# RWKV/rwkv.cpp

Measured on AMD Instinct MI355X. Metric: tokens/sec single-stream decode, higher is better.
Workload: dtype int8 x int4 dot, f32 accumulate (Q4_0 weights, Q8_0 activations); f16 head; 1 GPU; RWKV-6-World-7B Q4_0 single-stream greedy decode, state resident in HBM; layers=32, n_embed=4096, n_vocab=65536, parallelism=1 GPU, persist_kind=2

## Files before the change

### rwkv.cpp_amd/csrc/ring_geom.h

```cpp
#pragma once

#include <stdint.h>

#if defined(__HIPCC__)
#define RG_HD __host__ __device__ inline
#else
#define RG_HD inline
#endif

namespace rwkvmi {

constexpr int RG_NBLK = 256;
constexpr int RG_NC = 6;
constexpr int RG_CHUNK = 1024;

enum { RG_W1 = 0, RG_C = 1, RG_DW1 = 2, RG_E = 3, RG_FK = 4, RG_FR = 5, RG_G = 6, RG_NPHASE = 7 };

struct RingShape {
    int D, F, R5, DR;
    int qs, scb, qhb;
    int bal = 0;
};

constexpr int RG_BAL_C_N[3] = {5, 7, 4};
// ... 89 lines not shown
        if (j0 < c.n[p]) return c.off[p] + j0 * c.rec[p];
    }
    return RG_NONE;
}

constexpr int RG_HSTEPS = 8;
constexpr uint32_t RG_HREC = RG_HSTEPS * 1024;
struct RingHead { int hg, chunks, passes; uint32_t bytes; };
RG_HD RingHead rg_head(int n_vocab, int K) {
    RingHead h;
    h.hg = n_vocab / (RG_NBLK * 16);
    h.chunks = K / 32 / RG_HSTEPS;
    h.passes = (h.hg + RG_NC - 1) / RG_NC;
    h.bytes = (uint32_t) h.hg * (uint32_t) h.chunks * RG_HREC;
    return h;
}
RG_HD int rg_head_npc(const RingHead & h, int pass) { const int r = h.hg - RG_NC * pass; return r < RG_NC ? r : RG_NC; }
RG_HD uint32_t rg_head_off(const RingHead & h, int pass, int chunk, int cons) {
    return ((uint32_t) (RG_NC * pass * h.chunks) + (uint32_t) (chunk * rg_head_npc(h, pass) + cons)) * RG_HREC;
}

RG_HD int rg_x_rows(const RingShape & s, int cons) { const int n = rg_rows_e(s); return cons < n ? (n - cons + RG_NC - 1) / RG_NC : 0; }

}
```

### rwkv.cpp_amd/csrc/ring_v6.hip

```cpp
#include "persist.h"
#include "ring_geom.h"

namespace rwkvmi {

struct R6Cu { unsigned long long base; unsigned chunks, chunks_head; unsigned layer_bytes, pad; };

struct R6P {
    const M6Layer * layers; int n_layers;
    const unsigned char * arena;
    const float * w2b;
    float * x;
    float * x_out;
    const float * sin; float * sout; long long state_stride;
    void * xch; unsigned xch_bytes;
    int tl, act5, rkvg, dl, yq, xatt, kq, xffn;
    int act_stride;
    unsigned * ctl;
    const unsigned char * stream; const R6Cu * cus;
    int layer0, layers_total;
    int F, DR, R, H;
    int head_wg0;
    unsigned ring_bytes, mirror_bytes;
    int inflight, thin;
    int look;
    int look_g;
    int hthin;
    int nap;
    int burst;
    int dbg;
    float * logits; long long lnout_w, lnout_b; int n_vocab;
    const unsigned * tok; unsigned * next_tok; const void * emb; int emb_f16; long long ln0_w, ln0_b; int am;
    long long * trace; int trace_layer;
};

enum { FL_LANDED = 0, FL_SWB = 1, FL_SWE = 2 , FL_DONE = 4 , FL_GX = 12, FL_GACT = 13, FL_GYQ = 14, FL_GKQ = 15,
       FL_RED1 = 16, FL_RED2 = 17, FL_PRO = 18, FL_KEYS = 19,
       FL_HX = 20, FL_HACT = 21, FL_HYQ = 22, FL_HKQ = 23, FL_HTL = 24 ,
       FL_PROX = 25 ,
       FL_HWB = 26, FL_HWE = 27 ,
       FL_XRQ = 28 ,
       FL_AM = 29 , FL_WORDS = 32 };

struct R6Lds { size_t x, q1, q2, u, tl, bc, red, out, dl, misc, fl, ring, fixed; };
__host__ __device__ inline R6Lds r6_lds(int D, int F) {
    R6Lds o; size_t p = 0;
    auto take = [&](size_t n) { const size_t r = p; p += (n + 15) / 16 * 16; return r; };
    o.x = take((size_t) D * 4); o.q1 = take(qvec_bytes(D)); o.q2 = take(qvec_bytes(D));
    const size_t ua = 3 * ((qvec_bytes(D) + 15) / 16 * 16), ub = qvec_bytes(F);
    o.u = take(ua > ub ? ua : ub);
    o.tl = take(5 * 64 * 4); o.bc = take(64 * 16); o.red = take(2 * 256 * 8); o.out = take(64 * 4); o.dl = take(qvec_bytes(256)); o.misc = take(64);
    o.fl = take(FL_WORDS * 4);
    p = (p + 1023) / 1024 * 1024;
    o.ring = p; o.fixed = p;
    return o;
}

__device__ __forceinline__ unsigned fl_ld(unsigned * f) { return __builtin_amdgcn_readfirstlane(__hip_atomic_load(f, __ATOMIC_RELAXED, __HIP_MEMORY_SCOPE_WORKGROUP)); }
__device__ __forceinline__ void fl_st(unsigned * f, unsigned v) { asm volatile("" ::: "memory"); if ((threadIdx.x & 63) == 0) __hip_atomic_store(f, v, __ATOMIC_RELAXED, __HIP_MEMORY_SCOPE_WORKGROUP); }
__device__ __forceinline__ void fl_add(unsigned * f, unsigned v) { asm volatile("" ::: "memory"); if ((threadIdx.x & 63) == 0) (void) __hip_atomic_fetch_add(f, v, __ATOMIC_RELAXED, __HIP_MEMORY_SCOPE_WORKGROUP); }

__device__ __forceinline__ bool lds_backoff(Poll & pl, unsigned spin) {
    if ((spin & 1023u) == 1023u) {
        if (__hip_atomic_load(pl.ctl + 1, __ATOMIC_RELAXED, __HIP_MEMORY_SCOPE_AGENT) != 0u) pl.dead = true;
        else if (spin > 60000000u) { __hip_atomic_store(pl.ctl + 1, 2u, __ATOMIC_RELAXED, __HIP_MEMORY_SCOPE_AGENT); pl.dead = true; }
    }
    __builtin_amdgcn_s_sleep(1);
    return pl.dead;
}
__device__ __forceinline__ void fl_wait(Poll & pl, unsigned * f, unsigned want) {
    for (unsigned spin = 0;; spin++) {
        if (fl_ld(f) >= want || pl.dead) break;
        if (lds_backoff(pl, spin)) break;
    }
    asm volatile("" ::: "memory");
}

template <int FMT> struct RBlk { wv4i q[QF<FMT>::QS / 16]; unsigned qh, sc; };
template <int FMT, int R, int U> struct RawRec { RBlk<FMT> raw[U][R]; };
// ... 557 lines not shown
        for (int o = 32; o > 0; o >>= 1) { const float ov = __shfl_xor(best, o, WAVE); const int oi = __shfl_xor(bi, o, WAVE); am_merge(best, bi, ov, oi); }
    }

#ifndef R6_DMA_OFFSET_BOTH
#define R6_DMA_OFFSET_BOTH 1
#endif
    template <bool NT>
    static __device__ __forceinline__ void dma_quad(unsigned long long sbase, unsigned voff, unsigned m0dst) {
        unsigned keep;
#if R6_DMA_OFFSET_BOTH
#define R6_QUAD(POL) "s_mov_b32 %0, m0\n\ts_mov_b32 m0, %3\n\ts_nop 0\n\t" \
                     "global_load_lds_dwordx4 %1, %2" POL "\n\tglobal_load_lds_dwordx4 %1, %2 offset:1024" POL "\n\t" \
                     "global_load_lds_dwordx4 %1, %2 offset:2048" POL "\n\tglobal_load_lds_dwordx4 %1, %2 offset:3072" POL "\n\ts_mov_b32 m0, %0"
#else
#define R6_QUAD(POL) "s_mov_b32 %0, m0\n\ts_mov_b32 m0, %3\n\ts_nop 0\n\t" \
                     "global_load_lds_dwordx4 %1, %2" POL "\n\ts_add_u32 m0, m0, 0x400\n\ts_nop 0\n\tglobal_load_lds_dwordx4 %1, %2 offset:1024" POL "\n\t" \
                     "s_add_u32 m0, m0, 0x400\n\ts_nop 0\n\tglobal_load_lds_dwordx4 %1, %2 offset:2048" POL "\n\t" \
                     "s_add_u32 m0, m0, 0x400\n\ts_nop 0\n\tglobal_load_lds_dwordx4 %1, %2 offset:3072" POL "\n\ts_mov_b32 m0, %0"
#endif
        if constexpr (NT) asm volatile(R6_QUAD(" nt") : "=&s"(keep) : "v"(voff), "s"(sbase), "s"(m0dst) : "memory");
        else asm volatile(R6_QUAD("") : "=&s"(keep) : "v"(voff), "s"(sbase), "s"(m0dst) : "memory");
#undef R6_QUAD
    }
    static __device__ __forceinline__ void wait_vm(int w) {
        switch (w >> 2) {
            case 0:  asm volatile("s_waitcnt vmcnt(0)" ::: "memory"); break;
            case 1:  asm volatile("s_waitcnt vmcnt(4)" ::: "memory"); break;
            case 2:  asm volatile("s_waitcnt vmcnt(8)" ::: "memory"); break;
            case 3:  asm volatile("s_waitcnt vmcnt(12)" ::: "memory"); break;
            case 4:  asm volatile("s_waitcnt vmcnt(16)" ::: "memory"); break;
            case 5:  asm volatile("s_waitcnt vmcnt(20)" ::: "memory"); break;
            case 6:  asm volatile("s_waitcnt vmcnt(24)" ::: "memory"); break;
            case 7:  asm volatile("s_waitcnt vmcnt(28)" ::: "memory"); break;
            case 8:  asm volatile("s_waitcnt vmcnt(32)" ::: "memory"); break;
            case 9:  asm volatile("s_waitcnt vmcnt(36)" ::: "memory"); break;
            case 10: asm volatile("s_waitcnt vmcnt(40)" ::: "memory"); break;
            case 11: asm volatile("s_waitcnt vmcnt(44)" ::: "memory"); break;
            case 12: asm volatile("s_waitcnt vmcnt(48)" ::: "memory"); break;
            default: asm volatile("s_waitcnt vmcnt(52)" ::: "memory"); break;
        }
    }
    static __device__ __forceinline__ void loader_main(const R6P & p, const Lds & l, int lane) {
        const int wave = 0;
        const R6Cu cu = p.cus[blockIdx.x];
        unsigned total_ = p.logits ? cu.chunks_head : cu.chunks;
        if (p.n_layers != p.layers_total) {
            const unsigned long long bytes = (unsigned long long) p.n_layers * cu.layer_bytes + (p.logits ? (unsigned long long) rg_head(p.n_vocab, D).bytes : 0ull);
            total_ = (unsigned) ((bytes + 4 * RG_CHUNK - 1) / (4 * RG_CHUNK)) * 4u;
        }
        const unsigned total = __builtin_amdgcn_readfirstlane(total_);
        const unsigned long long src0 = (unsigned long long) p.stream + cu.base + (unsigned long long) p.layer0 * cu.layer_bytes;
        const unsigned RB = __builtin_amdgcn_readfirstlane(p.ring_bytes), MIR = __builtin_amdgcn_readfirstlane(p.mirror_bytes);
        const unsigned ring_m0 = __builtin_amdgcn_readfirstlane((unsigned) (size_t) (__attribute__((address_space(3))) unsigned char *) l.ring);
        const unsigned voff = (unsigned) lane * 16u;
        const int w_norm = __builtin_amdgcn_readfirstlane(p.inflight) & ~3, w_thin = __builtin_amdgcn_readfirstlane(p.thin) & ~3, w_hint = __builtin_amdgcn_readfirstlane(p.hthin) & ~3;
        Poll pl{p.ctl, false};
        unsigned issued = 0, roff = 0, landed = 0;
        unsigned min_done = 0, thin = 0;
        int level = 0;
        const unsigned burst = (unsigned) __builtin_amdgcn_readfirstlane(p.burst);
        const unsigned s_lo = __builtin_amdgcn_readfirstlane((unsigned) src0), s_hi = __builtin_amdgcn_readfirstlane((unsigned) (src0 >> 32));
        const int li = p.trace_layer;
        R6STAMP(0);
        unsigned stalls = 0, rounds = 0;
        unsigned long long sb = ((unsigned long long) s_hi << 32) | s_lo;
        unsigned * const fland = l.fl + FL_LANDED;
        long long * const lsamp = (p.trace && (blockIdx.x == 0 || blockIdx.x == 131)) ? p.trace + (size_t) gridDim.x * 8 * 32 + (blockIdx.x == 0 ? 0 : 2048) : nullptr;
        const unsigned samp_lo = (unsigned) p.trace_layer * cu.layer_bytes, samp_hi = samp_lo + cu.layer_bytes;
        unsigned nsamp = 0;
        for (unsigned spin = 0; issued < total;) {
            const unsigned lim0 = min_done >= total * 1024u ? total : ((min_done + RB) >> 12) << 2;
            const unsigned lim = lim0 < total ? lim0 : total;
            asm volatile("" ::: "memory");
            const v4u da = *reinterpret_cast<const v4u *>(l.fl + FL_DONE), db = *reinterpret_cast<const v4u *>(l.fl + FL_DONE + 4);
            const v4u dh = *reinterpret_cast<const v4u *>(l.fl);
            const uint2 dw = *reinterpret_cast<const uint2 *>(l.fl + FL_HWB);
            const int w = thin == 1u ? w_thin : (thin == 2u ? w_hint : w_norm);
            rounds++;
            if (lsamp && nsamp < 512u && issued * 1024u + 4096u > samp_lo && landed * 1024u < samp_hi) {
                if (lane == 0) {
                    long long * o = lsamp + (size_t) nsamp * 4;
                    o[0] = (long long) __builtin_amdgcn_s_memrealtime(); o[1] = (long long) issued * 1024 - samp_lo; o[2] = (long long) landed * 1024 - samp_lo;
                    o[3] = (long long) min_done - samp_lo;
                }
                nsamp++;
            }
            if (issued < lim) {
                spin = 0;
                unsigned n = (lim - issued) >> 2;
                n = n < burst ? n : burst;
                for (unsigned k = 0; k < n; k++) {
                    if (roff < MIR) { dma_quad<false>(sb, voff, ring_m0 + RB + roff); dma_quad<true>(sb, voff, ring_m0 + roff); level += 8; }
                    else { dma_quad<true>(sb, voff, ring_m0 + roff); level += 4; }
                    sb += 4096ull;
                    roff += 4096u; roff = roff >= RB ? 0u : roff;
                }
                issued += 4u * n;
                if (level > w) { wait_vm(w); level = w; }
            } else {
                stalls++;
                if (level > 0) { const int x = (level - 1) & ~3; wait_vm(x); level = x; }
                else if (lds_backoff(pl, spin++)) break;
            }
            {
                const unsigned ld = issued > (unsigned) level ? issued - (unsigned) level : 0u;
                if (ld > landed) { landed = ld; asm volatile("" ::: "memory"); __hip_atomic_store(fland, landed, __ATOMIC_RELAXED, __HIP_MEMORY_SCOPE_WORKGROUP); }
            }
            {
                unsigned m = da.x < da.y ? da.x : da.y; m = m < da.z ? m : da.z; m = m < da.w ? m : da.w;
                m = m < db.x ? m : db.x; m = m < db.y ? m : db.y; m = m < db.z ? m : db.z; m = m < db.w ? m : db.w;
                min_done = __builtin_amdgcn_readfirstlane(m);
                thin = __builtin_amdgcn_readfirstlane(dh.y != dh.z ? 1u : (dw.x != dw.y ? 2u : 0u));
            }
        }
        wait_vm(0);
        fl_st(l.fl + FL_LANDED, total);
        R6STAMP(1);
        if (p.trace && lane == 0) {
            p.trace[((long long) blockIdx.x * 8 + wave) * 32 + 2] = (long long) stalls;
            p.trace[((long long) blockIdx.x * 8 + wave) * 32 + 3] = (long long) rounds;
        }
    }

    struct Cons {
        RingCu cu;
        unsigned lbase;
        unsigned next_block;
        unsigned RB;
        unsigned ring_lds;
        unsigned landed;
        int c, lane;
        int dbg;
        unsigned look;
        long long waited;
    };
    template <int T, int TE> struct Unroll {
        template <typename F> static __device__ __forceinline__ void run(F && f) { f(std::integral_constant<int, T>{}); Unroll<T + 1, TE>::run(f); }
    };
    template <int TE> struct Unroll<TE, TE> { template <typename F> static __device__ __forceinline__ void run(F &&) {} };

    template <int PH, int R, int U, int NP> struct Pre {
        static constexpr int PH_ = PH, R_ = R, U_ = U, NP_ = NP;
        static constexpr unsigned RECB = (unsigned) (U * R * 64) * (QF<FMT>::QS + (QF<FMT>::HM ? 4 : 2) + (QF<FMT>::QH ? 4 : 0));
        RawRec<FMT, R, U> w[NP];
        unsigned have;
        unsigned cnt;
        unsigned pos, ro;
        unsigned after;
        unsigned base;
    };
    template <int PH, int T>
    static __device__ __forceinline__ unsigned ownj(const Cons & cs) {
// ... 18 lines not shown
        const unsigned nxt = rg_next_own_in_layer(cs.cu, cs.c, PH + 1);
        pre.after = __builtin_amdgcn_readfirstlane(nxt != RG_NONE ? cs.lbase + nxt : cs.next_block);
#pragma unroll
        for (int i = 0; i < NP; i++) rec_reserve<FMT, R, U>(pre.w[i]);
    }
    template <int T, int PH, int R, int U, int NP, bool WAIT = true>
    static __device__ __forceinline__ bool rec_take(Cons & cs, Poll & pl, const Lds & l, Pre<PH, R, U, NP> & pre, bool block) {
        constexpr unsigned RECB = recb<R, U>(), STRIDE = NC * RECB;
        const unsigned need = (pre.pos + RECB + 1023u) >> 10;
        if (cs.landed < need) {
            cs.landed = fl_ld(l.fl + FL_LANDED);
            if (cs.landed < need) {
                if (!block) return false;
                const long long t0 = (long long) __builtin_readcyclecounter();
                for (unsigned spin = 0;; spin++) {
                    cs.landed = fl_ld(l.fl + FL_LANDED);
                    if (cs.landed >= need || pl.dead) break;
                    if (lds_backoff(pl, spin)) break;
                }
                cs.waited += (long long) __builtin_readcyclecounter() - t0;
            }
        }
        asm volatile("" ::: "memory");
        rec_load<FMT, R, U>(pre.w[T % NP], cs.ring_lds, pre.ro, opq(cs.lane));
        asm volatile("" ::: "memory");
        const bool last = pre.have + 1u >= pre.cnt;
        unsigned nxt;
        if constexpr (balph<PH>()) nxt = pre.base + ownj<PH, T + 1>(cs) * RECB; else nxt = pre.pos + STRIDE;
        __hip_atomic_store(l.fl + FL_DONE + 2 + cs.c, last ? pre.after : nxt, __ATOMIC_RELAXED, __HIP_MEMORY_SCOPE_WORKGROUP);
        if constexpr (WAIT) rec_wait<FMT, R, U>(pre.w[T % NP]);
        pre.have += 1u;
        pre.ro += nxt - pre.pos; pre.pos = nxt;
        pre.ro = pre.ro >= cs.RB ? pre.ro - cs.RB : pre.ro;
        if constexpr (!balph<PH>() && STRIDE > 32768u) { pre.ro = pre.ro >= cs.RB ? pre.ro - cs.RB : pre.ro; pre.ro = pre.ro >= cs.RB ? pre.ro - cs.RB : pre.ro; }
        return true;
    }
#ifndef R6_PRE_MASK
#define R6_PRE_MASK 255
#endif
#ifndef R6_PRE_MASK_SMALL
#define R6_PRE_MASK_SMALL 255
#endif
    static constexpr int PRE_MASK = EPT > 4 ? R6_PRE_MASK : R6_PRE_MASK_SMALL;
    template <int PA_, int RA, int UA, int NA, int PB_, int RB_, int UB_, int NB_, int PC_, int RC, int UC, int NC_>
    static __device__ __forceinline__ void hint_take(Cons & cs, Poll & pl, const Lds & l, xrsrc xr, int unit, unsigned tag, unsigned * go, unsigned gen, int nap,
                                                     bool on_a, Pre<PA_, RA, UA, NA> & a, bool on_b, Pre<PB_, RB_, UB_, NB_> & b, bool on_c, Pre<PC_, RC, UC, NC_> & c3, bool no_handover = false) {
// ... 112 lines not shown
#ifndef R6_NPC
#define R6_NPC (Q8 ? 3 : (Q5 ? 5 : 6))
#endif
#ifndef R6_NPE
#define R6_NPE 3
#endif
#ifndef R6_NPK
#define R6_NPK ((PRE_MASK & 128) ? (Q8 ? 2 : (Q5 ? 4 : 5)) : (Q8 ? 3 : (Q5 ? 5 : 6)))
#endif
#ifndef R6_NPG
#define R6_NPG (Q8 ? 1 : 3)
#endif
    static constexpr int NPC = npcap((PRE_MASK & 1) ? R6_NPC : (Q8 ? 1 : 2), TFC);
    static constexpr int NPE = npcap((PRE_MASK & 2) ? R6_NPE : (Q8 ? 1 : 2), TFE);
    static constexpr int NPK = npcap((PRE_MASK & 4) ? R6_NPK : (Q8 ? 1 : 2), TFK);
    static constexpr int NPR = npcap((PRE_MASK & 128) ? 3 : (Q8 ? 1 : 2), TFE);
    static constexpr int NPG = npcap((PRE_MASK & 8) ? R6_NPG : 1, TFE);
#ifndef R6_G_PRE_OLD
#define R6_G_PRE_OLD 0
#endif
    static constexpr int rec_regs(int R, int U) { return U * R * (QF<FMT>::QS / 4 + 1 + (QF<FMT>::QH ? 1 : 0)); }
    static constexpr bool G_PRE = R6_G_PRE_OLD ? sizeof(RawRec<FMT, 1, UF>) <= 48 * 4 : rec_regs(1, UF) <= 48;

    static __device__ __forceinline__ void consumer_main(const R6P & p, const Lds & l, int lane, int wave, unsigned base) {
        const int blk = blockIdx.x;
        const int c = wave - 2;
        const bool pro = c < 4 || SHI > 0;
        const int F = p.F, nbF = F / 32;
        Poll pl{p.ctl, false, p.xch, R6_SWATCH == 1};
        const M6Arena ar{p.arena};
        const xrsrc xr = make_xrsrc(p.xch, p.xch_bytes);
        const RingShape sh = shape(p);
        Cons cs;
        cs.cu = rg_cu(sh, blk); cs.lbase = 0; cs.landed = 0; cs.RB = __builtin_amdgcn_readfirstlane(p.ring_bytes); cs.ring_lds = __builtin_amdgcn_readfirstlane((unsigned) (size_t) (__attribute__((address_space(3))) unsigned char *) l.ring); cs.c = c; cs.lane = lane; cs.dbg = __builtin_amdgcn_readfirstlane(p.dbg); cs.look = (unsigned) __builtin_amdgcn_readfirstlane(p.look); cs.waited = 0;
        const int mat = (blk * (4 * D / NBLK)) / D;
        const int cbase = (blk * (4 * D / NBLK)) % D;
        const bool has_dw1 = blk < p.DR;

        const unsigned first_own = rg_next_own_in_layer(cs.cu, c, 0);
        const RingHead hd = rg_head(p.n_vocab, D);
        const unsigned hbase = (unsigned) p.n_layers * cs.cu.layer_bytes;
        const unsigned head_first = (p.logits && c < hd.hg) ? hbase + rg_head_off(hd, 0, 0, c) : 0xFFFFFFFFu;
        float xown[XT], rrow[XT];
#pragma unroll
        for (int t = 0; t < XT; t++) { const int row = c + NC * t; xown[t] = row < RE ? p.x[blk * RE + row] : 0.0f; rrow[t] = 0.0f; }
        const bool emb_in = p.tok != nullptr;
        const unsigned eg = emb_in ? 1u : 0u;
        if (emb_in && c < 4) embed_ln0(p, pl, l, ar, c * 64 + opq(lane), opq(lane));
#ifndef R6_LATE_PARAMS
#define R6_LATE_PARAMS 2
#endif
        constexpr bool PA_EARLY = R6_LATE_PARAMS == 0 || (R6_LATE_PARAMS == 2 && (PRE_MASK & 16) == 0);
        constexpr bool PF_EARLY = R6_LATE_PARAMS == 0 || (R6_LATE_PARAMS == 2 && (PRE_MASK & 4) == 0);
        PA pa; PF pf;
        if (PA_EARLY) issue_pa(pa, ar, p.layers[0], p.sin, c, opq(lane));

        for (int li = 0; li < p.n_layers; li++) {
            const M6Layer & L = p.layers[li];
            const float * sin_l = p.sin + (long long) li * p.state_stride;
            float * sout_l = p.sout + (long long) li * p.state_stride;
            const unsigned tagL = base + (unsigned) li * 8u;
            const unsigned g1 = (unsigned) li + 1u;
            cs.lbase = (unsigned) li * cs.cu.layer_bytes;
            cs.next_block = li + 1 < p.n_layers ? cs.lbase + cs.cu.layer_bytes + first_own : head_first;
            R6STAMP(0);
            if (p.trace && li == p.trace_layer && lane == 0) p.trace[((long long) blockIdx.x * 8 + wave) * 32 + 23] = cs.waited;
            unsigned havepk = 0u;
            Pre<RG_W1, 1, UD, 1> pw;
            pre_begin<RG_W1>(cs, pw);
            Pre<RG_C, 2, UD, NPC> pc;
            pre_begin<RG_C>(cs, pc);
            {
                const bool first = li == 0;
                watch_begin(l);
                hint_take(cs, pl, l, xr, p.xffn + ((blk * 37 + c * 211) & 1023), tagL - 8u + SLOT_XFFN, l.fl + FL_HX, 2u * li + 1u, p.nap, (PRE_MASK & 16) != 0 && !first, pw,
                          (PRE_MASK & 16) != 0 && !first, pc, first);
                watch_end(l);
                if (R6_LATE_PARAMS == 2 && !PA_EARLY) { issue_pa(pa, ar, L, sin_l, c, opq(lane)); __builtin_amdgcn_sched_barrier(0); }
                sweep_begin(l);
                gather_x(pl, xr, p.xffn, tagL - 8u + SLOT_XFFN, c, opq(lane), l.x, first ? p.x : nullptr, first && emb_in);
            }
            gather_meet(pl, l.fl + FL_GX, 2u * li + 1u);
            sweep_end(l);
            R6STAMP(1);
            {
                const bool take = li == 0 && emb_in;
#pragma unroll
                for (int t = 0; t < XT; t++) { const int row = c + NC * t; const float v = l.x[blk * RE + (row < RE ? row : 0)]; xown[t] = take ? v : xown[t]; }
            }
            if (R6_LATE_PARAMS == 1) { issue_pa(pa, ar, L, sin_l, c, opq(lane)); __builtin_amdgcn_sched_barrier(0); }
            if (pro) prologue_A(pl, l, pa, sout_l, blk == 0, c, opq(lane), 2u * li + 1u, eg);
            prologue_wait(pl, l, 2u * li + 1u);
            R6STAMP(2);
            havepk |= pw.have;
            rows<RG_W1, 1, UD, 0, 1>(cs, pl, l, qvec_at(l.q1, D), nb, pw, [&](auto, int j, const float (&res)[1]) {
                if (lane == 0) tg_store(xr, p.tl + blk + NBLK * j, __float_as_uint(det_tanhf(res[0])), 0u, 0u, 0u, tagL + SLOT_TL);
            });
            R6STAMP(3);
            Pre<RG_E, 1, UD, NPE> pe;
            pre_begin<RG_E>(cs, pe);
            {
                const int img = (0x4213 >> (4 * mat)) & 0xF;
// ... 61 lines not shown
            sweep_end(l);
            R6STAMP(8);
            if (R6_LATE_PARAMS == 1) { issue_pf(pf, ar, L, sin_l, c, opq(lane)); __builtin_amdgcn_sched_barrier(0); }
            if (pro) prologue_F(pl, l, pf, sout_l, blk == 0, c, opq(lane), 2u * li + 2u, eg);
            prologue_wait(pl, l, 2u * li + 2u);
            R6STAMP(9); R6RSTAMP(28);
            if (p.trace && li == p.trace_layer && lane == 0) p.trace[((long long) blockIdx.x * 8 + wave) * 32 + 21] = (long long) fl_ld(l.fl + FL_LANDED) * 1024ll - (long long) (cs.lbase + cs.cu.off[RG_FK]);
            havepk |= (pk.have << 12) | (pr.have << 16);
            rows<RG_FK, 2, UD, TFK, NPK, TMK>(cs, pl, l, qvec_at(l.q1, D), nb, pk, [&](auto, int j, const float (&res)[2]) {
                const float v = lane == 1 ? res[1] : res[0];
                const float t = v > 0.0f ? v : 0.0f;
                if (lane < 2) l.out[2 * j + lane] = t * t;
            });
            fl_add(l.fl + FL_KEYS, 1u);
            if constexpr (DEFER_XR) {
                if (pro) quant_xr(l, c, opq(lane));
                fl_wait(pl, l.fl + FL_XRQ, (unsigned) (SHI > 0 ? NC : 4) * g1);
            }
            R6STAMP(10);
            rows<RG_FR, 1, UD, RE / NC, NPR>(cs, pl, l, qvec_at(l.q2, D), nb, pr, [&](auto tc, int, const float (&res)[1]) {
                constexpr int t = decltype(tc)::value;
                rrow[t] = res[0];
            });
            R6STAMP(11); R6RSTAMP(29);
            Pre<RG_G, 1, UF, NPG> pg;
            pre_begin<RG_G>(cs, pg);
            watch_begin(l);
            { const unsigned lk = cs.look; cs.look = (unsigned) __builtin_amdgcn_readfirstlane(p.look_g);
              hint_take(cs, pl, l, xr, p.kq + ((blk * 5 + c * 173) & 511), tagL + SLOT_KQ, l.fl + FL_HKQ, g1, p.nap, (PRE_MASK & 8) != 0 && G_PRE, pg);
              cs.look = lk; }
            watch_end(l);
            sweep_begin(l);
            gather_qvec<KSL>(pl, xr, p.kq, F, tagL + SLOT_KQ, c, opq(lane), l.kq);
            gather_meet(pl, l.fl + FL_GKQ, g1);
            sweep_end(l);
            R6STAMP(12); R6RSTAMP(30);
            if (p.trace && li == p.trace_layer && lane == 0) p.trace[((long long) blockIdx.x * 8 + wave) * 32 + 22] = (long long) fl_ld(l.fl + FL_LANDED) * 1024ll - (long long) (cs.lbase + cs.cu.off[RG_G]);
            havepk |= pg.have << 20;
            rows<RG_G, 1, UF, RE / NC, NPG>(cs, pl, l, qvec_at(l.kq, F), nbF, pg, [&](auto tc, int j, const float (&res)[1]) {
                constexpr int t = decltype(tc)::value;
                const float gte = sigmoid_f(rrow[t]) * res[0];
                xown[t] = xown[t] + gte;
                if (li == p.n_layers - 1 && lane == 0) p.x_out[blk * RE + j] = xown[t];
            });
            if (lane == 0) tg_store(xr, p.xffn + blk * NC + c, __float_as_uint(xown[0]), __float_as_uint(xown[XT > 1 ? 1 : 0]), __float_as_uint(xown[XT > 2 ? 2 : 0]), 0u, tagL + SLOT_XFFN);
            R6STAMP(13); R6RSTAMP(14);
            if (p.trace && li == p.trace_layer && lane == 0) { p.trace[((long long) blockIdx.x * 8 + wave) * 32 + 25] = cs.waited; p.trace[((long long) blockIdx.x * 8 + wave) * 32 + 15] = (long long) havepk; }
            __builtin_amdgcn_sched_barrier(0);
            if (PA_EARLY) {
                const int nl = li + 1 < p.n_layers ? li + 1 : li;
                issue_pa(pa, ar, p.layers[nl], p.sin + (long long) nl * p.state_stride, c, opq(lane));
            }
            __builtin_amdgcn_sched_barrier(0);
        }
        if (p.logits) head_phase(p, l, cs, pl, xr, ar, hd, hbase, lane, wave, base, eg);
    }

    static __device__ __forceinline__ void head_phase(const R6P & p, const Lds & l, Cons & cs, Poll & pl, xrsrc xr, const M6Arena & ar, const RingHead & hd,
                                                      unsigned hbase, int lane, int wave, unsigned base, unsigned eg) {
        const int blk = blockIdx.x, c = cs.c, li = p.n_layers;
        const unsigned tagL = base + (unsigned) li * 8u;
        const int pt = c * 64 + lane;
        R6STAMP(0); R6RSTAMP(16);
        watch_begin(l);
        gather_hint(pl, xr, p.xffn + ((blk * 37 + c * 211) & 1023), tagL - 8u + SLOT_XFFN, l.fl + FL_HX, 2u * li + 1u, p.nap);
        watch_end(l);
        sweep_begin(l);
        gather_x(pl, xr, p.xffn, tagL - 8u + SLOT_XFFN, c, opq(lane), l.x);
        gather_meet(pl, l.fl + FL_GX, 2u * li + 1u);
        sweep_end(l);
        R6STAMP(1);
        if (c < 4) {
            const float scale = ln_stats(pl, l, pt, lane, 2u * li + 1u + eg);
            const float * lw = ar.f(p.lnout_w), * lb = ar.f(p.lnout_b);
#pragma unroll
            for (int u = 0; u < (D + 1023) / 1024; u++) {
                const int i = pt * 4 + u * 1024;
                if (i >= D) break;
                const float4 xc = *reinterpret_cast<const float4 *>(l.x + i);
                const float4 w4 = *reinterpret_cast<const float4 *>(lw + i), b4 = *reinterpret_cast<const float4 *>(lb + i);
                const float xs[4] = {xc.x, xc.y, xc.z, xc.w}, ws[4] = {w4.x, w4.y, w4.z, w4.w}, bs[4] = {b4.x, b4.y, b4.z, b4.w};
                float y[4];
#pragma unroll
                for (int j = 0; j < 4; j++) { const float a = xs[j] * scale; const float aw = a * ws[j]; y[j] = round_f16(aw + bs[j]); }
                *reinterpret_cast<float4 *>(l.x + i) = make_float4(y[0], y[1], y[2], y[3]);
            }
            fl_add(l.fl + FL_PRO, 1u);
        }
        fl_wait(pl, l.fl + FL_PRO, 4u * (2u * li + 1u));
        R6STAMP(2);
// ... 67 lines not shown
        fl_add(l.fl + FL_AM, 1u);
        R6STAMP(7); R6RSTAMP(17);
        if (p.trace && li == p.trace_layer && lane == 0) p.trace[((long long) blockIdx.x * 8 + wave) * 32 + 21] = waited;
    }

    static __device__ __forceinline__ void comm_main(const R6P & p, const Lds & l, int lane, unsigned base) {
        const int wave = 1;
        const int blk = blockIdx.x;
        const int g = NC;
        const int F = p.F, DR = p.DR, R = p.R, H = p.H;
        const int nbF = F / 32;
        Poll pl{p.ctl, false, p.xch, R6_SWATCH != 0};
        const M6Arena ar{p.arena};
        const xrsrc xr = make_xrsrc(p.xch, p.xch_bytes);
        const int mat = (blk * (4 * D / NBLK)) / D;
        const bool has_dw1 = blk < DR;
        const int hw0 = __builtin_amdgcn_readfirstlane(p.head_wg0);
        const bool d_has = blk >= hw0 && blk < hw0 + H;
        const int d_head = blk - hw0;
        const int gpb = (nbF + NBLK - 1) / NBLK;
        constexpr int NCH = 5 * (D / 64);
        const int b_extra = NCH - NBLK;
        const int b_chunk2 = (b_extra > 0 && blk >= NBLK / 4 && blk < NBLK / 4 + b_extra) ? NBLK + (blk - NBLK / 4) : -1;

        for (int li = 0; li < p.n_layers; li++) {
            const M6Layer & L = p.layers[li];
            const float * sin_l = p.sin + (long long) li * p.state_stride;
            float * sout_l = p.sout + (long long) li * p.state_stride;
            const unsigned tagL = base + (unsigned) li * 8u;
            const unsigned g1 = (unsigned) li + 1u;
            R6STAMP(0);
            {
                const bool first = li == 0;
                watch_begin(l);
                if (!first) gather_hint(pl, xr, p.xffn + ((blk * 37 + g * 211) & 1023), tagL - 8u + SLOT_XFFN, l.fl + FL_HX, 2u * li + 1u, p.nap);
                watch_end(l);
                sweep_begin(l);
                gather_x(pl, xr, p.xffn, tagL - 8u + SLOT_XFFN, g, opq(lane), l.x, first ? p.x : nullptr, first && p.tok != nullptr);
            }
            gather_meet(pl, l.fl + FL_GX, 2u * li + 1u);
            sweep_end(l);
            R6STAMP(1); R6RSTAMP(17);
            const int lnA = opq(lane);
            float4 wB4[2][16]; float wBmaa[2], cw[2], cb_[2], cpv[2];
            int bf[2], bd[2];
#pragma unroll
            for (int q = 0; q < 2; q++) {
                const int ch = q == 0 ? (blk < NCH ? blk : 0) : (b_chunk2 >= 0 ? b_chunk2 : 0);
                bf[q] = ch / (D / 64);
                bd[q] = (ch % (D / 64)) * 64 + lnA;
                const float4 * cbp = reinterpret_cast<const float4 *>(p.w2b + L.w2b + (long long) ch * R * 64);
#pragma unroll
                for (int m4 = 0; m4 < 16; m4++) { const int4 t = ldw16(cbp + (m4 < R / 4 ? m4 : R / 4 - 1) * 64 + lnA); wB4[q][m4] = make_float4(__int_as_float(t.x), __int_as_float(t.y), __int_as_float(t.z), __int_as_float(t.w)); }
                wBmaa[q] = ar.f(L.maa[bf[q]])[bd[q]];
                cw[q] = ar.f(L.ln1_w)[bd[q]]; cb_[q] = ar.f(L.ln1_b)[bd[q]]; cpv[q] = sin_l[D + bd[q]];
            }
            RawRec<FMT, 1, UD> dwr;
            {
                const WPl dw1 = ar.w(L.dw1);
                const int drow = has_dw1 ? blk : 0;
// ... 197 lines not shown
            gather_hint(pl, xr, p.xatt + ((blk * 37 + g * 211) & 1023), tagL + SLOT_XATT, l.fl + FL_HX, 2u * li + 2u, p.nap);
            watch_end(l);
            sweep_begin(l);
            gather_x(pl, xr, p.xatt, tagL + SLOT_XATT, g, opq(lane), l.x);
            gather_meet(pl, l.fl + FL_GX, 2u * li + 2u);
            sweep_end(l);
            R6STAMP(8); R6RSTAMP(23);
            if constexpr (KCOMM > 0) {
                if (k_has) {
                    prologue_wait(pl, l, 2u * li + 2u);
                    const int lnK = opq(lane);
                    ActRegs<UD> ark;
                    act_load<FMT, UD>(ark, qvec_at(l.q1, D), nb, lnK);
                    float part[2 * KCOMM];
#pragma unroll
                    for (int q = 0; q < KCOMM; q++) rec_acc<FMT, 2, UD>(kxr[q], ark, nb, lnK, part + 2 * q);
                    wave_sum_n<2 * KCOMM>(part);
                    const float v = pick_lane<2 * KCOMM>(part, lnK);
                    const float t = v > 0.0f ? v : 0.0f;
                    if (lnK < 2 * KCOMM) l.out[2 * (KSETS - KCOMM) + lnK] = t * t;
                    __builtin_amdgcn_wave_barrier();
                }
            }
            fl_wait(pl, l.fl + FL_KEYS, (unsigned) NC * g1);
            R6STAMP(9);
            {
                const int ln = opq(lane);
                for (int g2 = 0; g2 < (gpb + 1) / 2; g2++) {
                    const int gi = g2 * 2 + (ln >> 5);
                    const int gg = blk * gpb + gi;
                    const bool valid = gi < gpb && gg < nbF;
                    const float v = valid ? l.out[gi * 32 + (ln & 31)] : 0.0f;
                    int qi, isum; float d16, s16;
                    quant_block32(v, qi, d16, s16, isum);
                    tq_store_block(xr, p.kq, valid ? gg : 0, ln & 31, qi, d16, s16, isum, tagL + SLOT_KQ, valid);
                }
            }
            R6STAMP(10); R6RSTAMP(24);
            watch_begin(l);
            gather_hint(pl, xr, p.kq + ((blk * 5 + g * 173) & 511), tagL + SLOT_KQ, l.fl + FL_HKQ, g1, p.nap);
            watch_end(l);
            sweep_begin(l);
            gather_qvec<KSL>(pl, xr, p.kq, F, tagL + SLOT_KQ, g, opq(lane), l.kq);
            gather_meet(pl, l.fl + FL_GKQ, g1);
            sweep_end(l);
            R6STAMP(11); R6RSTAMP(25);
        }
        if (p.logits) {
            const int li = p.n_layers;
            const unsigned tagL = base + (unsigned) li * 8u;
            watch_begin(l);
            gather_hint(pl, xr, p.xffn + ((blk * 37 + g * 211) & 1023), tagL - 8u + SLOT_XFFN, l.fl + FL_HX, 2u * li + 1u, p.nap);
            watch_end(l);
            sweep_begin(l);
            gather_x(pl, xr, p.xffn, tagL - 8u + SLOT_XFFN, g, opq(lane), l.x);
            gather_meet(pl, l.fl + FL_GX, 2u * li + 1u);
            sweep_end(l);
        }
        tail_argmax(p, l, pl, xr, opq(lane), base);
    }

    static __device__ __forceinline__ void tail_argmax(const R6P & p, const Lds & l, Poll & pl, xrsrc xr, int lane, unsigned base) {
        const int blk = blockIdx.x;
        const unsigned tagA = base + (unsigned) (p.n_layers - 1) * 8u + 7u;
        float b = -INFINITY; int bi = 0x7fffffff;
        if (p.logits) {
            fl_wait(pl, l.fl + FL_AM, (unsigned) NC);
            if (lane < NC) { b = l.bc[2 * lane]; bi = __float_as_int(l.bc[2 * lane + 1]); }
            am_wave(b, bi);
        }
        if (lane == 0) tg_store(xr, p.am + blk, __float_as_uint(b), (unsigned) bi, 0u, 0u, tagA);
        if (!p.logits || !p.next_tok || blk != 0) return;
        int ptr[NBLK / 64]; bool valid[NBLK / 64]; v4u dv[NBLK / 64];
#pragma unroll
        for (int k = 0; k < NBLK / 64; k++) { ptr[k] = p.am + lane + 64 * k; valid[k] = true; }
        poll_ptrs<NBLK / 64>(pl, xr, ptr, valid, tagA, dv);
        float b3 = -INFINITY; int i3 = 0x7fffffff;
// ... 102 lines not shown
        const int col = 32 * (k * RG_HSTEPS + st) + 8 * q;
        const int4 v = *reinterpret_cast<const int4 *>(head + row * K + col);
        *reinterpret_cast<int4 *>(dst + st * 1024 + lane * 16) = v;
    }
}

__global__ void k_block_w2_ring(const float * __restrict__ src, float * __restrict__ dst, int D, int R) {
    const long long n = 5ll * R * D;
    for (long long i = (long long) blockIdx.x * blockDim.x + threadIdx.x; i < n; i += (long long) gridDim.x * blockDim.x) {
        const int d = (int) (i % D); const long long fm = i / D; const int m = (int) (fm % R), f = (int) (fm / R);
        const long long o = ((((long long) f * (D / 64) + d / 64) * (R / 4) + m / 4) * 64 + d % 64) * 4 + m % 4;
        dst[o] = src[i];
    }
}

struct RingShared {
    int ref = 0;
    float * w2b = nullptr;
    M6Layer * d_layers = nullptr;
    R6Cu * d_cus = nullptr;
    unsigned char * stream = nullptr;
    int variant = -1, n_blocks = 0, n_layers = 0;
    size_t lds = 0, ring = 0, mirror = 0;
    uint64_t bytes = 0;
    bool head = false;
    uint64_t bytes_head = 0;
    bool embed = false;
    uint64_t bytes_embed = 0;
    long long lnw_off = 0, lnb_off = 0, ln0w_off = 0, ln0b_off = 0;
    int64_t D = 0, F = 0, DR = 0, R = 0;
};

struct RingV6 : PersistentDecoder {
    const Model * model = nullptr;
    RingShared * sh = nullptr;
    void * xch = nullptr;
    R6P proto{};

    ~RingV6() override;
    DecodePath kind() const override { return DecodePath::Ring; }
    uint64_t bytes() const override { return sh->bytes; }
    bool folds_embed() const override { return sh->embed; }
    bool folds_head() const override { return sh->head; }
    bool folds_argmax() const override { return sh->head; }
    void forward_range(float * x, float * v_first, const float * sin, float * sout, hipStream_t st, DecodeProf * pf, float * logits, int l0, int l1,
                       const uint32_t * tok, uint32_t * next_tok) override;
// ... 55 lines not shown
    if (hipGetDeviceProperties(&prop, m.device) != hipSuccess) return nullptr;
    const int NB = prop.multiProcessorCount;
    const int v = ring_variant(m, NB);
    if (v < 0) return nullptr;
    const LayerW & L0 = m.layers[m.layer_begin];
    const int64_t D = m.n_embed(), F = L0.ffn_key->ne[1], DR = L0.att_time_decay_w1->ne[1], R = L0.att_time_maa_w1->ne[1] / 5;
    const int fmt = (int) m.header.data_type;
    RingShape sh; sh.D = (int) D; sh.F = (int) F; sh.R5 = (int) (5 * R); sh.DR = (int) DR;
    sh.qs = fmt == T_Q8_0 ? 32 : 16; sh.scb = (fmt == T_Q4_1 || fmt == T_Q5_1) ? 4 : 2; sh.qhb = (fmt == T_Q5_0 || fmt == T_Q5_1) ? 4 : 0;
    const int n_layers = (int) (m.layer_end - m.layer_begin);
    RingShared * rs = new RingShared();
    rs->variant = v; rs->n_blocks = NB; rs->n_layers = n_layers;
    rs->D = D; rs->F = F; rs->DR = DR; rs->R = R;
    const R6Lds lo = r6_lds((int) D, (int) F);
    const size_t lds_max = 160 * 1024;
    const size_t max_rec_bytes = rg_rec_bytes(sh, 1, (int) F) > rg_rec_bytes(sh, 2, (int) D) ? rg_rec_bytes(sh, 1, (int) F) : rg_rec_bytes(sh, 2, (int) D);
    const size_t mirror = ((max_rec_bytes > RG_HREC ? max_rec_bytes : RG_HREC) + 4095) / 4096 * 4096;
    size_t ring = (size_t) env_int("RWKV_MI_RING_KB", 1024) * 1024;
    if (lo.fixed + mirror + 32 * 1024 > lds_max) { delete rs; return nullptr; }
    if (ring > lds_max - lo.fixed - mirror) ring = lds_max - lo.fixed - mirror;
    ring = ring / 4096 * 4096;
    if (ring < 32 * 1024) ring = 32 * 1024;
    rs->lds = lo.fixed + ring + mirror; rs->ring = ring; rs->mirror = mirror;
    if (hipFuncSetAttribute((const void *) g_ring_variants[v].fn, hipFuncAttributeMaxDynamicSharedMemorySize, (int) rs->lds) != hipSuccess) { delete rs; return nullptr; }
    const bool fold_head = m.has_head && m.head && m.head->type == T_F16 && m.head->cols() == D && m.n_vocab() % (RG_NBLK * 16) == 0 && m.ln_out_w && m.ln_out_b
                           && !(getenv("RWKV_MI_RING_NO_HEAD") && getenv("RWKV_MI_RING_NO_HEAD")[0] == '1');
    rs->head = fold_head;
    std::vector<R6Cu> hc(RG_NBLK);
    uint64_t total = 0;
    int max_rec = 0;
    for (int b = 0; b < RG_NBLK; b++) {
        const RingCu cu = rg_cu(sh, b);
        int nr = 0; for (int ph = 0; ph < RG_NPHASE; ph++) nr += (int) cu.n[ph];
        max_rec = nr > max_rec ? nr : max_rec;
        const uint64_t bytes = (uint64_t) cu.layer_bytes * n_layers;
        if (bytes + (1u << 20) > 0xFFFFFFFFull) { delete rs; return nullptr; }
        const uint64_t hbytes = fold_head ? rg_head((int) m.n_vocab(), (int) D).bytes : 0;
        if (bytes + hbytes + (1u << 20) > 0xFFFFFFFFull) { delete rs; return nullptr; }
        hc[b].base = total; hc[b].chunks = (unsigned) ((bytes + 4 * RG_CHUNK - 1) / (4 * RG_CHUNK)) * 4u;
        hc[b].chunks_head = (unsigned) ((bytes + hbytes + 4 * RG_CHUNK - 1) / (4 * RG_CHUNK)) * 4u; hc[b].layer_bytes = cu.layer_bytes; hc[b].pad = 0;
        total += (uint64_t) hc[b].chunks_head * RG_CHUNK;
    }
    const size_t w2_layer = (size_t) 5 * R * D;
    bool ok = R % 4 == 0 && hipMalloc((void **) &rs->w2b, w2_layer * n_layers * sizeof(float)) == hipSuccess
           && hipMalloc((void **) &rs->stream, total + 4 * RG_CHUNK) == hipSuccess
           && hipMalloc((void **) &rs->d_cus, hc.size() * sizeof(R6Cu)) == hipSuccess
// ... 94 lines not shown
    const int64_t nbD = D / 32, nbF = F / 32;
    const int64_t PAD = 2048;
    auto up = [](int64_t v) { return (v + 63) / 64 * 64; };
    const int64_t act_stride = up(3 * nbD), xunits = up(RG_NBLK * RG_NC);
    const int64_t sizes[9] = {up(1280) + PAD, 5 * act_stride + PAD, 2 * D + PAD, 256 + PAD, act_stride + PAD, xunits + PAD, up(3 * nbF) + PAD, xunits + PAD, up(RG_NBLK) + PAD};
    int64_t units = 0;
    for (int64_t z : sizes) units += z;
    bool ok = hipMalloc(&rg->xch, (size_t) units * 16) == hipSuccess && hipMemset(rg->xch, 0, (size_t) units * 16) == hipSuccess
      && rg->ctl.alloc(8u);
    if (!ok || hipDeviceSynchronize() != hipSuccess) { delete rg; return nullptr; }
    R6P & q = rg->proto;
    q.layers = rs->d_layers; q.n_layers = rs->n_layers; q.layer0 = 0; q.layers_total = rs->n_layers;
    q.arena = (const unsigned char *) m.arena; q.w2b = rs->w2b;
    q.state_stride = m.state_per_layer();
    q.xch = rg->xch; q.xch_bytes = (unsigned) (units * 16);
    int u = 0;
    int * slots[9] = {&q.tl, &q.act5, &q.rkvg, &q.dl, &q.yq, &q.xatt, &q.kq, &q.xffn, &q.am};
    for (int i = 0; i < 9; i++) { *slots[i] = u; u += (int) sizes[i]; }
    q.act_stride = (int) act_stride;
    q.ctl = rg->ctl.dev;
    q.stream = rs->stream; q.cus = rs->d_cus;
    q.F = (int) F; q.DR = (int) rs->DR; q.R = (int) rs->R; q.H = (int) m.head_count;
    q.ring_bytes = (unsigned) rs->ring; q.mirror_bytes = (unsigned) rs->mirror;
    q.head_wg0 = env_int("RWKV_MI_RING_HEAD_WG", NB / 2);
    if (q.head_wg0 < 0 || q.head_wg0 + (int) m.head_count > NB) q.head_wg0 = 0;
    q.logits = nullptr; q.lnout_w = rs->lnw_off; q.lnout_b = rs->lnb_off; q.n_vocab = (int) m.n_vocab();
    q.tok = nullptr; q.next_tok = nullptr; q.emb = rs->embed ? m.emb->data : nullptr; q.emb_f16 = (rs->embed && m.emb->type == T_F16) ? 1 : 0; q.ln0_w = rs->ln0w_off; q.ln0_b = rs->ln0b_off;
    auto snap = [](int w) { w &= ~3; return w < 4 ? 4 : (w > 52 ? 52 : w); };
    q.inflight = snap(env_int("RWKV_MI_RING_INFLIGHT", 48));
    q.thin = snap(env_int("RWKV_MI_RING_THIN", 16));
    q.hthin = snap(env_int("RWKV_MI_RING_HTHIN", q.inflight));
    q.look = env_int("RWKV_MI_RING_LOOK", 1);
    if (q.look < 1) q.look = 1;
    q.look_g = env_int("RWKV_MI_RING_LOOKG", q.look);
    if (q.look_g < 1) q.look_g = 1;
    q.nap = env_int("RWKV_MI_RING_NAP", 2);
    q.dbg = env_int("RWKV_MI_RING_DBG", 0);
    q.burst = env_int("RWKV_MI_RING_BURST", 24) / 4;
    if (q.burst < 1) q.burst = 1;
    if (q.burst > 6) q.burst = 6;
    return rg;
}

void RingV6::forward_range(float * x, float *, const float * sin, float * sout, hipStream_t st, DecodeProf * pf, float * logits, int l0, int l1,
                           const uint32_t * tok, uint32_t * next_tok) {
    R6P q = proto;
// ... 13 lines not shown
```

Measured before the change: 645.9 tokens/s.

## Stage tail FFN value-matrix records into idle LDS scratch beyond the ring

Adds an extension buffer that reuses the x/q1/q2 LDS scratch region to hold the last few G-phase (FFN value) weight records of each layer, so the producer can prefetch them directly into that area instead of waiting for ring space. The producer DMAs those chunks into the extension region, gated by a new FL_XFREE counter that consumers bump once they stop using the scratch. Consumers read G records from the extension when past the offset, and wait on a drain check before gather_x overwrites the scratch. This lets more weight bytes be in flight across the layer boundary, at the cost of extra synchronization and the risk of LDS aliasing bugs.

```diff
diff --git a/rwkv.cpp_amd/csrc/ring_geom.h b/rwkv.cpp_amd/csrc/ring_geom.h
--- a/rwkv.cpp_amd/csrc/ring_geom.h
+++ b/rwkv.cpp_amd/csrc/ring_geom.h
@@ -1,5 +1,6 @@
 #pragma once
 
+#include <stddef.h>
 #include <stdint.h>
 
 #if defined(__HIPCC__)
@@ -135,4 +136,36 @@
 
 RG_HD int rg_x_rows(const RingShape & s, int cons) { const int n = rg_rows_e(s); return cons < n ? (n - cons + RG_NC - 1) / RG_NC : 0; }
 
+RG_HD size_t rg_qvec_bytes(int64_t K) { return (size_t) K + (size_t) (K / 32) * 12; }
+constexpr int RG_FL_WORDS = 32;
+struct R6Lds { size_t x, q1, q2, u, tl, bc, red, out, dl, misc, fl, ring, fixed; };
+RG_HD R6Lds r6_lds(int D, int F) {
+    R6Lds o; size_t p = 0;
+    auto take = [&](size_t n) { const size_t r = p; p += (n + 15) / 16 * 16; return r; };
+    o.x = take((size_t) D * 4); o.q1 = take(rg_qvec_bytes(D)); o.q2 = take(rg_qvec_bytes(D));
+    const size_t ua = 3 * ((rg_qvec_bytes(D) + 15) / 16 * 16), ub = rg_qvec_bytes(F);
+    o.u = take(ua > ub ? ua : ub);
+    o.tl = take(5 * 64 * 4); o.bc = take(64 * 16); o.red = take(2 * 256 * 8); o.out = take(64 * 4); o.dl = take(rg_qvec_bytes(256)); o.misc = take(64);
+    o.fl = take(RG_FL_WORDS * 4);
+    p = (p + 1023) / 1024 * 1024;
+    o.ring = p; o.fixed = p;
+    return o;
 }
+
+RG_HD uint32_t rg_ext_cap(const R6Lds & lo) { return (uint32_t) (lo.u - lo.x) / RG_CHUNK * RG_CHUNK; }
+RG_HD uint32_t rg_ext_recs(const RingShape & s, uint32_t cap, uint32_t ring_bytes) {
+    const uint32_t n = (uint32_t) rg_rows_e(s), rec = rg_rec_bytes(s, 1, s.F);
+    if (n * rec <= ring_bytes || cap < (uint32_t) RG_CHUNK) return 0u;
+    const uint32_t k = (cap - (uint32_t) (RG_CHUNK - 1)) / rec;
+    return k < n ? k : n;
+}
+RG_HD uint32_t rg_ext_off(const RingCu & c, uint32_t recs) { return recs ? c.off[RG_G] + (c.n[RG_G] - recs) * c.rec[RG_G] : RG_NONE; }
+RG_HD uint32_t rg_ext_lds(uint32_t pos, uint32_t xs) { return pos - (xs & ~(uint32_t) (RG_CHUNK - 1)); }
+enum { RG_TO_RING = 1, RG_TO_EXT = 2 };
+RG_HD int rg_chunk_dst(uint32_t ch, uint32_t xs, uint32_t xe) {
+    const uint32_t lo = ch * (uint32_t) RG_CHUNK, hi = lo + (uint32_t) RG_CHUNK;
+    if (hi <= xs || lo >= xe) return RG_TO_RING;
+    return RG_TO_EXT | ((lo < xs || hi > xe) ? RG_TO_RING : 0);
+}
+
+}
diff --git a/rwkv.cpp_amd/csrc/ring_v6.hip b/rwkv.cpp_amd/csrc/ring_v6.hip
--- a/rwkv.cpp_amd/csrc/ring_v6.hip
+++ b/rwkv.cpp_amd/csrc/ring_v6.hip
@@ -21,6 +21,7 @@
     int F, DR, R, H;
     int head_wg0;
     unsigned ring_bytes, mirror_bytes;
+    unsigned ext_recs;
     int inflight, thin;
     int look;
     int look_g;
@@ -39,21 +40,9 @@
        FL_PROX = 25 ,
        FL_HWB = 26, FL_HWE = 27 ,
        FL_XRQ = 28 ,
-       FL_AM = 29 , FL_WORDS = 32 };
-
-struct R6Lds { size_t x, q1, q2, u, tl, bc, red, out, dl, misc, fl, ring, fixed; };
-__host__ __device__ inline R6Lds r6_lds(int D, int F) {
-    R6Lds o; size_t p = 0;
-    auto take = [&](size_t n) { const size_t r = p; p += (n + 15) / 16 * 16; return r; };
-    o.x = take((size_t) D * 4); o.q1 = take(qvec_bytes(D)); o.q2 = take(qvec_bytes(D));
-    const size_t ua = 3 * ((qvec_bytes(D) + 15) / 16 * 16), ub = qvec_bytes(F);
-    o.u = take(ua > ub ? ua : ub);
-    o.tl = take(5 * 64 * 4); o.bc = take(64 * 16); o.red = take(2 * 256 * 8); o.out = take(64 * 4); o.dl = take(qvec_bytes(256)); o.misc = take(64);
-    o.fl = take(FL_WORDS * 4);
-    p = (p + 1023) / 1024 * 1024;
-    o.ring = p; o.fixed = p;
-    return o;
-}
+       FL_AM = 29 ,
+       FL_XFREE = 30 , FL_WORDS = RG_FL_WORDS };
+
 
 __device__ __forceinline__ unsigned fl_ld(unsigned * f) { return __builtin_amdgcn_readfirstlane(__hip_atomic_load(f, __ATOMIC_RELAXED, __HIP_MEMORY_SCOPE_WORKGROUP)); }
 __device__ __forceinline__ void fl_st(unsigned * f, unsigned v) { asm volatile("" ::: "memory"); if ((threadIdx.x & 63) == 0) __hip_atomic_store(f, v, __ATOMIC_RELAXED, __HIP_MEMORY_SCOPE_WORKGROUP); }
@@ -657,6 +646,12 @@
         else asm volatile(R6_QUAD("") : "=&s"(keep) : "v"(voff), "s"(sbase), "s"(m0dst) : "memory");
 #undef R6_QUAD
     }
+    template <bool NT>
+    static __device__ __forceinline__ void dma_one(unsigned long long sbase, unsigned voff, unsigned m0dst) {
+        unsigned keep;
+        if constexpr (NT) asm volatile("s_mov_b32 %0, m0\n\ts_mov_b32 m0, %3\n\ts_nop 0\n\tglobal_load_lds_dwordx4 %1, %2 nt\n\ts_mov_b32 m0, %0" : "=&s"(keep) : "v"(voff), "s"(sbase), "s"(m0dst) : "memory");
+        else asm volatile("s_mov_b32 %0, m0\n\ts_mov_b32 m0, %3\n\ts_nop 0\n\tglobal_load_lds_dwordx4 %1, %2\n\ts_mov_b32 m0, %0" : "=&s"(keep) : "v"(voff), "s"(sbase), "s"(m0dst) : "memory");
+    }
     static __device__ __forceinline__ void wait_vm(int w) {
         switch (w >> 2) {
             case 0:  asm volatile("s_waitcnt vmcnt(0)" ::: "memory"); break;
@@ -700,6 +695,9 @@
         unsigned stalls = 0, rounds = 0;
         unsigned long long sb = ((unsigned long long) s_hi << 32) | s_lo;
         unsigned * const fland = l.fl + FL_LANDED;
+        unsigned xq0 = 0xFFFFFFFFu;
+        if (!(__builtin_amdgcn_readfirstlane(p.dbg) & 8) && p.ext_recs != 0u)
+            xq0 = __builtin_amdgcn_readfirstlane(((cu.layer_bytes - p.ext_recs * rg_rec_bytes(shape(p), 1, p.F)) >> 12) << 2);
         long long * const lsamp = (p.trace && (blockIdx.x == 0 || blockIdx.x == 131)) ? p.trace + (size_t) gridDim.x * 8 * 32 + (blockIdx.x == 0 ? 0 : 2048) : nullptr;
         const unsigned samp_lo = (unsigned) p.trace_layer * cu.layer_bytes, samp_hi = samp_lo + cu.layer_bytes;
         unsigned nsamp = 0;
@@ -720,10 +718,44 @@
                 }
                 nsamp++;
             }
-            if (issued < lim) {
+            if (issued >= xq0) {
+                const unsigned LB = __builtin_amdgcn_readfirstlane(p.cus[blockIdx.x].layer_bytes);
+                const unsigned xl = (issued * 1024u) / LB, xe = (xl + 1u) * LB, xs = xe - p.ext_recs * rg_rec_bytes(shape(p), 1, p.F);
+                int dall = 0;
+#pragma unroll 1
+                for (unsigned j = 0; j < 4u; j++) dall |= rg_chunk_dst(issued + j, xs, xe);
+                const bool xgo = (!(dall & RG_TO_RING) || issued + 4u <= lim) && fl_ld(l.fl + FL_XFREE) >= (unsigned) NG * (xl + 1u);
+                if (xgo) {
+                    spin = 0;
+                    const unsigned xc0 = xs >> 10;
+                    const unsigned ext_m0 = (unsigned) (size_t) (__attribute__((address_space(3))) unsigned char *) (unsigned char *) l.x;
+#pragma unroll 1
+                    for (unsigned j = 0; j < 4u; j++) {
+                        const unsigned ch = issued + j;
+                        const int d = rg_chunk_dst(ch, xs, xe);
+                        const unsigned long long sj = sb + 1024ull * j;
+                        if (d & RG_TO_EXT) { if (d & RG_TO_RING) dma_one<false>(sj, voff, ext_m0 + (ch - xc0) * 1024u); else dma_one<true>(sj, voff, ext_m0 + (ch - xc0) * 1024u); level += 1; }
+                        if (d & RG_TO_RING) {
+                            const unsigned rj = roff + 1024u * j;
+                            if (rj < MIR) { dma_one<false>(sj, voff, ring_m0 + RB + rj); level += 1; }
+                            dma_one<true>(sj, voff, ring_m0 + rj); level += 1;
+                        }
+                    }
+                    sb += 4096ull;
+                    roff += 4096u; roff = roff >= RB ? 0u : roff;
+                    issued += 4u;
+                    if (issued * 1024u >= xe) xq0 = xl + 1u < (unsigned) p.n_layers ? ((xs + LB) >> 12) << 2 : 0xFFFFFFFFu;
+                    if (level > w) { wait_vm(w); level = w; }
+                } else {
+                    stalls++;
+                    if (level > 0) { const int x = (level - 1) & ~3; wait_vm(x); level = x; }
+                    else if (lds_backoff(pl, spin++)) break;
+                }
+            } else if (issued < lim) {
                 spin = 0;
                 unsigned n = (lim - issued) >> 2;
                 n = n < burst ? n : burst;
+                { const unsigned nx = (xq0 - issued) >> 2; n = n < nx ? n : nx; }
                 for (unsigned k = 0; k < n; k++) {
                     if (roff < MIR) { dma_quad<false>(sb, voff, ring_m0 + RB + roff); dma_quad<true>(sb, voff, ring_m0 + roff); level += 8; }
                     else { dma_quad<true>(sb, voff, ring_m0 + roff); level += 4; }
@@ -763,6 +795,7 @@
         unsigned next_block;
         unsigned RB;
         unsigned ring_lds;
+        unsigned xoff;
         unsigned landed;
         int c, lane;
         int dbg;
@@ -827,6 +860,11 @@
             }
         }
         asm volatile("" ::: "memory");
+        if constexpr (PH == RG_G) {
+            const bool inx = pre.pos - cs.lbase >= cs.xoff;
+            const unsigned ext_lds = (unsigned) (size_t) (__attribute__((address_space(3))) unsigned char *) (unsigned char *) l.x;
+            rec_load<FMT, R, U>(pre.w[T % NP], inx ? ext_lds : cs.ring_lds, inx ? rg_ext_lds(pre.pos, cs.lbase + cs.xoff) : pre.ro, opq(cs.lane));
+        } else
         rec_load<FMT, R, U>(pre.w[T % NP], cs.ring_lds, pre.ro, opq(cs.lane));
         asm volatile("" ::: "memory");
         const bool last = pre.have + 1u >= pre.cnt;
@@ -985,6 +1023,18 @@
     static constexpr int rec_regs(int R, int U) { return U * R * (QF<FMT>::QS / 4 + 1 + (QF<FMT>::QH ? 1 : 0)); }
     static constexpr bool G_PRE = R6_G_PRE_OLD ? sizeof(RawRec<FMT, 1, UF>) <= 48 * 4 : rec_regs(1, UF) <= 48;
 
+    static __device__ __forceinline__ void ext_drained(Poll & pl, const Lds & l, unsigned upto) {
+        for (unsigned spin = 0;; spin++) {
+            asm volatile("" ::: "memory");
+            const v4u da = *reinterpret_cast<const v4u *>(l.fl + FL_DONE), db = *reinterpret_cast<const v4u *>(l.fl + FL_DONE + 4);
+            unsigned m = da.z < da.w ? da.z : da.w;
+            m = m < db.x ? m : db.x; m = m < db.y ? m : db.y; m = m < db.z ? m : db.z; m = m < db.w ? m : db.w;
+            if (__builtin_amdgcn_readfirstlane(m) >= upto || pl.dead) break;
+            if (lds_backoff(pl, spin)) break;
+        }
+        asm volatile("" ::: "memory");
+    }
+
     static __device__ __forceinline__ void consumer_main(const R6P & p, const Lds & l, int lane, int wave, unsigned base) {
         const int blk = blockIdx.x;
         const int c = wave - 2;
@@ -996,6 +1046,7 @@
         const RingShape sh = shape(p);
         Cons cs;
         cs.cu = rg_cu(sh, blk); cs.lbase = 0; cs.landed = 0; cs.RB = __builtin_amdgcn_readfirstlane(p.ring_bytes); cs.ring_lds = __builtin_amdgcn_readfirstlane((unsigned) (size_t) (__attribute__((address_space(3))) unsigned char *) l.ring); cs.c = c; cs.lane = lane; cs.dbg = __builtin_amdgcn_readfirstlane(p.dbg); cs.look = (unsigned) __builtin_amdgcn_readfirstlane(p.look); cs.waited = 0;
+        cs.xoff = __builtin_amdgcn_readfirstlane(rg_ext_off(cs.cu, p.ext_recs));
         const int mat = (blk * (4 * D / NBLK)) / D;
         const int cbase = (blk * (4 * D / NBLK)) % D;
         const bool has_dw1 = blk < p.DR;
@@ -1041,6 +1092,7 @@
                 watch_end(l);
                 if (R6_LATE_PARAMS == 2 && !PA_EARLY) { issue_pa(pa, ar, L, sin_l, c, opq(lane)); __builtin_amdgcn_sched_barrier(0); }
                 sweep_begin(l);
+                if (cs.xoff != RG_NONE) ext_drained(pl, l, cs.lbase);
                 gather_x(pl, xr, p.xffn, tagL - 8u + SLOT_XFFN, c, opq(lane), l.x, first ? p.x : nullptr, first && emb_in);
             }
             gather_meet(pl, l.fl + FL_GX, 2u * li + 1u);
@@ -1148,6 +1200,7 @@
                 constexpr int t = decltype(tc)::value;
                 rrow[t] = res[0];
             });
+            if (cs.xoff != RG_NONE) fl_add(l.fl + FL_XFREE, 1u);
             R6STAMP(11); R6RSTAMP(29);
             Pre<RG_G, 1, UF, NPG> pg;
             pre_begin<RG_G>(cs, pg);
@@ -1192,6 +1245,7 @@
         gather_hint(pl, xr, p.xffn + ((blk * 37 + c * 211) & 1023), tagL - 8u + SLOT_XFFN, l.fl + FL_HX, 2u * li + 1u, p.nap);
         watch_end(l);
         sweep_begin(l);
+        if (cs.xoff != RG_NONE) ext_drained(pl, l, hbase);
         gather_x(pl, xr, p.xffn, tagL - 8u + SLOT_XFFN, c, opq(lane), l.x);
         gather_meet(pl, l.fl + FL_GX, 2u * li + 1u);
         sweep_end(l);
@@ -1305,6 +1359,8 @@
         constexpr int NCH = 5 * (D / 64);
         const int b_extra = NCH - NBLK;
         const int b_chunk2 = (b_extra > 0 && blk >= NBLK / 4 && blk < NBLK / 4 + b_extra) ? NBLK + (blk - NBLK / 4) : -1;
+        const unsigned xrecs = (unsigned) __builtin_amdgcn_readfirstlane(p.ext_recs);
+        const unsigned layer_bytes = __builtin_amdgcn_readfirstlane(p.cus[blk].layer_bytes);
 
         for (int li = 0; li < p.n_layers; li++) {
             const M6Layer & L = p.layers[li];
@@ -1319,6 +1375,7 @@
                 if (!first) gather_hint(pl, xr, p.xffn + ((blk * 37 + g * 211) & 1023), tagL - 8u + SLOT_XFFN, l.fl + FL_HX, 2u * li + 1u, p.nap);
                 watch_end(l);
                 sweep_begin(l);
+                if (xrecs) ext_drained(pl, l, (unsigned) li * layer_bytes);
                 gather_x(pl, xr, p.xffn, tagL - 8u + SLOT_XFFN, g, opq(lane), l.x, first ? p.x : nullptr, first && p.tok != nullptr);
             }
             gather_meet(pl, l.fl + FL_GX, 2u * li + 1u);
@@ -1562,6 +1619,7 @@
                     __builtin_amdgcn_wave_barrier();
                 }
             }
+            if (xrecs) fl_add(l.fl + FL_XFREE, 1u);
             fl_wait(pl, l.fl + FL_KEYS, (unsigned) NC * g1);
             R6STAMP(9);
             {
@@ -1593,6 +1651,7 @@
             gather_hint(pl, xr, p.xffn + ((blk * 37 + g * 211) & 1023), tagL - 8u + SLOT_XFFN, l.fl + FL_HX, 2u * li + 1u, p.nap);
             watch_end(l);
             sweep_begin(l);
+            if (xrecs) ext_drained(pl, l, (unsigned) li * layer_bytes);
             gather_x(pl, xr, p.xffn, tagL - 8u + SLOT_XFFN, g, opq(lane), l.x);
             gather_meet(pl, l.fl + FL_GX, 2u * li + 1u);
             sweep_end(l);
@@ -1741,6 +1800,7 @@
     unsigned char * stream = nullptr;
     int variant = -1, n_blocks = 0, n_layers = 0;
     size_t lds = 0, ring = 0, mirror = 0;
+    unsigned ext_recs = 0;
     uint64_t bytes = 0;
     bool head = false;
     uint64_t bytes_head = 0;
@@ -1842,6 +1902,8 @@
     ring = ring / 4096 * 4096;
     if (ring < 32 * 1024) ring = 32 * 1024;
     rs->lds = lo.fixed + ring + mirror; rs->ring = ring; rs->mirror = mirror;
+    if (rg_qvec_bytes(D) != qvec_bytes(D) || rg_qvec_bytes(F) != qvec_bytes(F)) { delete rs; return nullptr; }
+    rs->ext_recs = env_int("RWKV_MI_RING_EXT", 1) != 0 ? rg_ext_recs(sh, rg_ext_cap(lo), (uint32_t) ring) : 0u;
     if (hipFuncSetAttribute((const void *) g_ring_variants[v].fn, hipFuncAttributeMaxDynamicSharedMemorySize, (int) rs->lds) != hipSuccess) { delete rs; return nullptr; }
     const bool fold_head = m.has_head && m.head && m.head->type == T_F16 && m.head->cols() == D && m.n_vocab() % (RG_NBLK * 16) == 0 && m.ln_out_w && m.ln_out_b
                            && !(getenv("RWKV_MI_RING_NO_HEAD") && getenv("RWKV_MI_RING_NO_HEAD")[0] == '1');
@@ -1982,6 +2044,7 @@
     q.stream = rs->stream; q.cus = rs->d_cus;
     q.F = (int) F; q.DR = (int) rs->DR; q.R = (int) rs->R; q.H = (int) m.head_count;
     q.ring_bytes = (unsigned) rs->ring; q.mirror_bytes = (unsigned) rs->mirror;
+    q.ext_recs = rs->ext_recs;
     q.head_wg0 = env_int("RWKV_MI_RING_HEAD_WG", NB / 2);
     if (q.head_wg0 < 0 || q.head_wg0 + (int) m.head_count > NB) q.head_wg0 = 0;
     q.logits = nullptr; q.lnout_w = rs->lnw_off; q.lnout_b = rs->lnb_off; q.n_vocab = (int) m.n_vocab();
```

Measured after the change: 547.1 tokens/s. -15.3%, worse.
